# DiltheyLab/MetaMaps

Measured on AMD Instinct MI355X. Metric: Gbp long reads mapped+classified per sec (whole node), miniSeq+H DB, higher is better.
Workload: dtype u32

## Files before the change

metamaps_amd/csrc/mm_env.hpp:

```cpp
#pragma once
#include <unistd.h>
#include <cstdlib>
#include <cstring>
#include <string>

extern "C" char** environ;

namespace mm {

struct EnvSwitch { const char* name; const char* dflt; const char* kind; const char* what; };

inline const EnvSwitch* env_table(size_t* n) {
  static const EnvSwitch T[] = {
    {"MM_STRICT_ENV", "unset", "user", "refuse MM_* variables that are not in this table (mm_ctx_create returns MM_ERR_ARG, the CLI exits 1)"},
    {"MM_CPU_BUDGET", "min(hardware threads, affinity mask, cgroup CPU quota)", "user", "CPUs the process may keep busy: what every thread pool of the library and the CLI is sized from (cpu_budget.hpp)"},
    {"MM_SYNC", "block when the CPU budget is <= 32, else spin", "user", "how a host thread waits for its stream: \"spin\" (hipStreamSynchronize) or \"block\" (sleep on an event created with hipEventBlockingSync)"},
    {"MM_CLI_WORKERS", "4", "user", "worker contexts per GPU that take read batches in turn (= --workers-per-gpu)"},
    {"MM_CLI_BATCH_READS", "100000", "user", "reads per batch handed to a worker"},
    {"MM_CLI_BATCH_MBASES", "256", "user", "... or this many million bases, whichever comes first"},
    {"MM_CLI_MAP_SLOTS", "2", "tuning", "batches per device that may be inside their mapping section at the same time"},
    {"MM_CLI_BLOCK_BYTES", "128 MiB", "tuning", "block size of the block-parallel FASTQ/FASTA parser over an mmap-ed query file"},
    {"MM_CLI_REF_BLOCK_BYTES", "min(group, 256 MiB)", "tuning", "the same for the reference FASTA"},
    {"MM_CLI_REF_GROUP_BASES", "2^30", "test", "bases per upload group of the reference (small groups: the concat path on small inputs)"},
    {"MM_CLI_REF_SEQUENTIAL", "unset", "test", "reference through the sequential kseq-style reader instead of the block parser"},
// ... 13 lines not shown
    {"MM_CLASSIFY_THREADS", "32", "user", "host threads that tokenise the mappings file and format classify's outputs"},
    {"MM_EM_MAX_ITER", "unbounded", "test", "cap on EM iterations in classify (the reference has none)"},
    {"MM_EM_SLICE", "1024", "test", "EM iterations per mm_em_run / mm_em_continue call of classify"},
    {"MM_CLI_TIMING", "unset", "debug", "phase laps of the CLI on stderr (bench.py's e2e legs parse them)"},
    {"MM_CLI_FORMAT_TRACE", "unset", "debug", "per-thread times of the text formatting of a batch on stderr"},
    {"MM_DEVICE_BYTES_CAP", "0 (off)", "test", "the library behaves as if every device had this many bytes: allocations beyond fail, mm_ctx_device_info reports it (placement tests)"},
    {"MM_INDEX_SCALE_MB", "8192", "test", "blocks from this size on are index-scale (pooled per device); a few MB exercise the pool on small inputs"},
    {"MM_NO_SLABS", "unset", "test", "worker buffers are not cut out of pooled index-scale blocks"},
    {"MM_NO_POOL_RESCUE", "unset", "test", "round-3 behaviour: a request the driver refuses hands the whole pool back instead of being served from it"},
    {"MM_ALLOC_TRACE", "unset", "debug", "every block that comes from the driver, with its cost, on stderr"},
    {"MM_CTX_TRACE", "unset", "debug", "phases of mm_ctx_create (HIP initialisation, stream, allocator) on stderr"},
    {"MM_HOST_TIMING", "unset", "debug", "host-side sections of mm_map_batch and of the index build on stderr"},
    {"MM_PACK_SCALAR", "unset", "test", "mm_seqset_upload packs bases with the byte-table loop only (cross-check of the AVX2 path, host_pack.cpp)"},
    {"MM_INDEX_PART_MAX", "2^31 - 2^24 entries", "test", "entries per partition of the hash sort (small values: the partitioned sort + merge on small inputs)"},
    {"MM_DUP_SAT", "65535", "test", "saturation value of the stored same-hash neighbour distances (small values: K5's scan fall-back)"},
    {"MM_EAGER_TIEBREAK", "unset", "test", "resolve every duplicate-hash strand by the reference's std::sort order up front instead of only where a strand vote reads one"},
    {"MM_FORCE_AMB_REDO", "unset", "test", "every read with an unresolved strand goes through the redo path"},
    {"MM_NO_HIT_FILTER", "unset", "test", "K3 without the exact seed-hit pre-filter: every hit of every kept list reaches the sort (parity tests of the raw hit list)"},
    {"MM_NO_FUSED_FILTER", "unset", "test", "K3 as probe_kernel + two-pass hit_filter_kernel for every read (what reads that do not fit the fused kernel take)"},
    {"MM_HF_STAGE_CAP", "auto", "test", "capacity of a read's survivor stage (tiny values: the overflow / re-filter path)"},
    {"MM_HF_WIDE_FROM", "13000", "tuning", "sketch size from which the two-pass filter counts in 32768 position slots instead of 8192"},
    {"MM_SEGSORT_MAX_KEYS", "2^32 - 1", "test", "keys per call of K4's segmented device sort (small values: the split on small inputs)"},
    {"MM_L1_SERIAL", "unset", "test", "K4's L1 merge loop as the literal one-thread-per-read loop (cross-check of the wavefront form)"},
    {"MM_L2_FULL", "unset", "test", "K5 evaluates every window (the literal slide) instead of the exact skip-ahead"},
    {"MM_L2_DENSE_FROM", "13000", "tuning", "sketch size from which K5 runs as l2_codes_kernel + l2_dense_kernel"},
    {"MM_L2_DENSE_NO_STOP", "unset", "test", "dense path without its early stop (every window evaluated)"},
    {"MM_L2_NO_SMALL_GROUPS", "unset", "test", "groups of fewer than three candidates also run as four-wave workgroups (one launch instead of two)"},
    {"MM_L2_HOST_GROUPS", "unset", "test", "candidate groups formed on the host instead of by l2_group_kernel"},
    {"MM_L2_NO_GROUP_SORT", "unset", "test", "K5 workgroups in read order instead of the order of their candidates' positions"},
    {"MM_L2_GROUP_SORT_MIN", "2048", "tuning", "groups from which the launch order is sorted"},
    {"MM_L2_V1", "unset", "test", "K5's 10 kb class through l2_kernel (rank codes per entry) instead of the zone kernel l2z_kernel (mm_l2z.hpp): the cross-check and the A/B"},
    {"MM_L2_V1_LONG", "unset", "test", "the long-read classes (sketches of 3 073 .. 13 000 hashes) through l2_kernel, the 10 kb class through the zone kernel"},
    {"MM_L2_NO_FUSE", "unset", "test", "zone kernel without the band predicted from L1's seed-hit count: its masks always come from a second pass over the stream"},
    {"MM_L2_NO_RANGES", "unset", "test", "the zone kernel's waves search their candidates' index ranges themselves (until round 6) instead of taking them from l2_ranges_kernel (cross-check)"},
    {"MM_L2Z_FORCE_HANDBACK", "unset", "test", "the zone kernel hands every candidate that reaches its band loop to l2_kernel, as its pass-count guard does (the hand-back path against the default)"},
    {"MM_L2Z_WALK_SEARCH", "unset", "test", "the 10 kb zone kernel finds the next block to sweep by the walk one block at a time (the long-read classes' way) instead of by ballots: the same blocks, the cross-check"},
    {"MM_L2Z_DBG", "unset", "debug", "zone kernel writes pivot-minus-estimate and its pass count INSTEAD OF RESULTS (tools/l2z_pivot_hist.py; 2: against the predicted estimate)"},
    {"MM_L2_ONE_STREAM", "unset", "test", "the two launches of K5's 10 kb class one behind the other on the context's stream instead of side by side (auxiliary stream)"},
    {"MM_L2_NO_SLOTS", "unset", "test", "K5 scratch indexed by wave number of the launch instead of per-XCD slots taken and given back"},
    {"MM_L2_SLOTS", "auto (resident waves)", "tuning", "number of K5 scratch slots"},
    {"MM_L2_STOP", "0", "debug", "K5 leaves after phase n WITHOUT RESULTS (tools/l2_stop.py)"},
    {"MM_L2_PHASES", "unset", "debug", "K5 phase clocks into its counters (tools/l2_long_phases.py; the zone kernel has them in a build with -DL2Z_CLOCKS only)"},
    {"MM_MZ_DBG", "0", "debug", "K1 leaves after step n WITHOUT RESULTS (tools/stage_ms.py)"},
    {"MM_HF_DBG", "0", "debug", "two-pass filter leaves after phase n WITHOUT RESULTS"},
    {"MM_SF_PROF", "unset", "debug", "cycle counts per phase of the streaming seed filter on stderr"},
    {"MM_EM_FORCE_COLLECTIVE", "unset", "test", "a one-rank communicator keeps P1-P3' | ncclAllReduce | finalize instead of P1-P3 alone (how one GPU drives the multi-rank path)"},
// ... 40 lines not shown
```

metamaps_amd/csrc/mm_l1.hpp:

```cpp
#pragma once
#include <rocprim/rocprim.hpp>
#include "mm_map.hpp"
#include "mm_l2.hpp"

namespace mm {

template <int IPT>
__global__ void __launch_bounds__(256) sort_hits_radix_kernel(uint64_t* __restrict__ hits, const uint64_t* __restrict__ read_hit_off,
                                                              const int32_t* __restrict__ read_list, int end_bit,
                                                              const uint64_t* __restrict__ stage ,
                                                              const uint64_t* __restrict__ stage_off ) {
  using Sort = rocprim::block_radix_sort<uint64_t, 256, IPT>;
  extern __shared__ __align__(16) unsigned char sort_dyn[];
  typename Sort::storage_type& tmp = *reinterpret_cast<typename Sort::storage_type*>(sort_dyn);
  const int r = read_list[blockIdx.x];
  const uint64_t o = read_hit_off[r];
  const int n = (int)(read_hit_off[r + 1] - o);
  const uint64_t* __restrict__ src = hits + o;
  if (stage) { const uint64_t sb = stage_off[r]; if ((uint64_t)n <= stage_off[r + 1] - sb) src = stage + sb; }
  uint64_t key[IPT];
#pragma unroll
  for (int i = 0; i < IPT; ++i) { const int idx = threadIdx.x * IPT + i; key[i] = idx < n ? src[idx] : ~0ull; }
  Sort().sort(key, tmp, 0, end_bit);
#pragma unroll
  for (int i = 0; i < IPT; ++i) { const int idx = threadIdx.x * IPT + i; if (idx < n) hits[o + idx] = key[i]; }
}

template <bool WRITE>
__global__ void l1_scan_kernel(const uint64_t* __restrict__ hits, const uint64_t* __restrict__ read_hit_off, const int32_t* __restrict__ read_len,
                               const int32_t* __restrict__ min_hits, int64_t n_reads, uint32_t* __restrict__ cand_n,
                               const uint64_t* __restrict__ cand_off, int32_t* __restrict__ cand, int32_t* __restrict__ cand_read) {
  int64_t r = (int64_t)blockIdx.x * blockDim.x + threadIdx.x;
  if (r >= n_reads) return;
  const uint64_t o = read_hit_off[r];
  const int64_t H = (int64_t)(read_hit_off[r + 1] - o);
  const int len = read_len[r];
  int m = min_hits[r]; if (m < 1) m = 1;
  uint32_t nc = 0;
  int lseq = -1, lstart = 0, lend = 0;
  uint64_t wbase = WRITE ? cand_off[r] : 0;
  auto flush = [&]() {
    if (lseq < 0) return;
    if (WRITE) { int32_t* c = cand + 3 * (wbase + nc); c[0] = lseq; c[1] = lstart; c[2] = lend; cand_read[wbase + nc] = (int32_t)r; }
    ++nc;
  };
  for (int64_t i = 0; i + m <= H; ++i) {
    uint64_t a = hits[o + i], b = hits[o + i + m - 1];
    int sa = (int)(a >> 32), sb = (int)(b >> 32);
    int wa = pw_wpos((uint32_t)a), wb = pw_wpos((uint32_t)b);
    if (sa != sb || wb - wa >= len) continue;
    int cs = max(0, wb - len + 1), ce = wa;
    if (lseq == sa && lend >= cs) lend = max(ce, lend);
    else { flush(); lseq = sa; lstart = cs; lend = ce; }
  }
  flush();
  if (!WRITE) cand_n[r] = nc;
}

template <bool WRITE>
__global__ void __launch_bounds__(256) l1_wave_kernel(const uint64_t* __restrict__ hits, const uint64_t* __restrict__ read_hit_off,
                                                      const int32_t* __restrict__ read_len, const int32_t* __restrict__ min_hits, int64_t n_reads,
                                                      uint32_t* __restrict__ cand_n, const uint64_t* __restrict__ cand_off, int32_t* __restrict__ cand,
                                                      int32_t* __restrict__ cand_read, int32_t* __restrict__ cand_hint ) {
  const int64_t r = (int64_t)blockIdx.x * 4 + (threadIdx.x >> 6);
  const int lane = threadIdx.x & 63;
  if (r >= n_reads) return;
  const uint64_t o = read_hit_off[r];
  const int64_t H = (int64_t)(read_hit_off[r + 1] - o);
  const int len = read_len[r];
  int m = min_hits[r]; if (m < 1) m = 1;
  const uint64_t wbase = WRITE ? cand_off[r] : 0;
  int count = 0, prev_seq = -1, prev_wa = 0;
  int64_t open_i = 0;
  for (int64_t base = 0; base + m <= H; base += 64) {
    const int64_t i = base + lane;
    const bool valid = i + m <= H;
    uint64_t a = 0, b = 0;
    if (valid) { a = hits[o + i]; b = hits[o + i + m - 1]; }
    const int sa = (int)(a >> 32), sb = (int)(b >> 32), wa = pw_wpos((uint32_t)a), wb = pw_wpos((uint32_t)b);
    const bool q = valid && sa == sb && wb - wa < len;
    const int cs = max(0, wb - len + 1);
    const uint64_t qm = __ballot(q);
    const uint64_t below = qm & ((1ull << lane) - 1ull);
    const int pl = below ? 63 - __builtin_clzll(below) : 0;
    const int p_seq_l = __shfl(sa, pl, 64), p_wa_l = __shfl(wa, pl, 64);
    const int p_seq = below ? p_seq_l : prev_seq, p_wa = below ? p_wa_l : prev_wa;
    const bool brk = q && !(p_seq == sa && p_wa >= cs);
    const uint64_t bm = __ballot(brk);
    if (WRITE && q) {
      const int k = count + __popcll(bm & ((2ull << lane) - 1ull)) - 1;
      const uint64_t above = lane < 63 ? qm & ~((2ull << lane) - 1ull) : 0ull;
      const bool last = above == 0ull || ((bm >> (__builtin_ctzll(above))) & 1ull);
      int32_t* c = cand + 3 * (wbase + (uint64_t)k);
      if (brk) { c[0] = sa; c[1] = cs; cand_read[wbase + (uint64_t)k] = (int32_t)r; }
      if (last) c[2] = wa;
      if (last && cand_hint) {
        const uint64_t opened = bm & ((2ull << lane) - 1ull);
        const int64_t oi = opened ? base + (63 - __builtin_clzll(opened)) : open_i;
        cand_hint[wbase + (uint64_t)k] = (int32_t)min((int64_t)0x7fffffff, i + m - oi);
      }
    }
    if (bm) open_i = base + (63 - __builtin_clzll(bm));
    count += __popcll(bm);
    if (qm) { const int ll = 63 - __builtin_clzll(qm); prev_seq = __shfl(sa, ll, 64); prev_wa = __shfl(wa, ll, 64); }
  }
  if (!WRITE && lane == 0) cand_n[r] = (uint32_t)count;
}

__global__ void __launch_bounds__(256) l2_group_kernel(const uint64_t* __restrict__ cand_off, const int32_t* __restrict__ sk_n, const int32_t* __restrict__ read_len,
                                                       int64_t n, int min_len_dense, int dense_from, int no_small,
                                                       int32_t* __restrict__ gA0, int32_t* __restrict__ gAn, int32_t* __restrict__ gS0, int32_t* __restrict__ gSn,
                                                       unsigned int* __restrict__ ctr) {
  __shared__ unsigned int bA, bS, bOther, bMax, baseA, baseS;
  if (threadIdx.x == 0) { bA = 0; bS = 0; bOther = 0; bMax = 0; }
  __syncthreads();
  const int64_t r = (int64_t)blockIdx.x * 256 + threadIdx.x;
  uint64_t c_lo = 0, c_hi = 0; int sr = 0; bool mine = false;
  if (r < n) {
    c_lo = cand_off[r]; c_hi = cand_off[r + 1]; sr = sk_n[r];
    const bool dense = sr >= dense_from && sr < L2_SKETCH_LIMIT && read_len[r] >= min_len_dense;
    mine = c_hi > c_lo && sr <= 3072 && !dense;
    if (c_hi > c_lo && !mine) atomicAdd(&bOther, 1u);
  }
  const unsigned ncr = mine ? (unsigned)(c_hi - c_lo) : 0u, nfull = ncr >> 2, rem = ncr & 3u;
  const bool rem_small = rem != 0 && rem <= 2 && !no_small;
  const unsigned a = nfull + ((rem != 0 && !rem_small) ? 1u : 0u), b = rem_small ? 1u : 0u;
  unsigned la = 0, ls = 0;
  if (a) la = atomicAdd(&bA, a);
  if (b) ls = atomicAdd(&bS, b);
// ... 82 lines not shown
```

metamaps_amd/csrc/mm_map.hip:

```cpp
#include "mm_map.hpp"
#include <functional>
#include <memory>
#include "mm_prims.hpp"
#include "mm_l2_core.hpp"
#include "mm_size_classes.hpp"
#include "mm_l2.hpp"
#include "mm_l2z.hpp"
#include "mm_l2_dense.hpp"
#include <cstdlib>
#include <atomic>
#include <thread>
#include "mm_stats.hpp"
#include <algorithm>
#include <numeric>
#include "mm_sketch.hpp"
#include "mm_seed.hpp"
#include "mm_l1.hpp"

namespace mm {

namespace {
struct HostLap {
  const bool on = getenv("MM_HOST_TIMING") != nullptr; std::chrono::steady_clock::time_point t = std::chrono::steady_clock::now();
  void operator()(const char* what) { if (!on) return; const auto n = std::chrono::steady_clock::now(); fprintf(stderr, "host %-28s %8.1f us\n", what, std::chrono::duration<double, std::micro>(n - t).count()); t = n; }
// ... 48 lines not shown
  std::vector<uint8_t> sv; std::vector<int32_t> scnt; std::atomic<int> mismatch{0};
  ~AmbState() { if (bg.joinable()) bg.join(); }
};

namespace {
struct MapSwitches {
  struct OptInt { bool set; int v; };
  static bool on(const char* e) { return e != nullptr; }
  static bool is1(const char* e) { return e && e[0] == '1'; }
  static int num(const char* e, int dflt) { return e ? atoi(e) : dflt; }
  static OptInt opt(const char* e) { return OptInt{e != nullptr, e ? atoi(e) : 0}; }
  const bool eager_tiebreak = on(getenv("MM_EAGER_TIEBREAK"));
  const bool use_filter = !is1(getenv("MM_NO_HIT_FILTER"));
  const bool use_fused = use_filter && !on(getenv("MM_NO_FUSED_FILTER"));
  const int hf_wide_env = num(getenv("MM_HF_WIDE_FROM"), 13000);
  const int hf_wide_from = hf_wide_env > 0 ? hf_wide_env : INT_MAX;
  const OptInt hf_stage_cap = opt(getenv("MM_HF_STAGE_CAP"));
  const int hf_dbg = num(getenv("MM_HF_DBG"), 0);
  const bool sf_prof = on(getenv("MM_SF_PROF"));
  const OptInt sf_grid = opt(getenv("MM_SF_GRID"));
  const OptInt segsort_max_env = opt(getenv("MM_SEGSORT_MAX_KEYS"));
  const uint64_t segsort_max_keys = segsort_max_env.set ? (uint64_t)std::max(segsort_max_env.v, 1) : 0xffffffffull;
  const bool l1_serial = on(getenv("MM_L1_SERIAL"));
  const bool l2_no_fuse = on(getenv("MM_L2_NO_FUSE"));
  const bool l2_no_ranges = on(getenv("MM_L2_NO_RANGES"));
  const bool l2_skip = !is1(getenv("MM_L2_FULL"));
  const int dense_from = num(getenv("MM_L2_DENSE_FROM"), 13000);
  const bool dense_no_stop = on(getenv("MM_L2_DENSE_NO_STOP"));
  const bool no_small_groups = on(getenv("MM_L2_NO_SMALL_GROUPS"));
  const bool dev_groups = l2_skip && !on(getenv("MM_L2_HOST_GROUPS"));
  const bool l2_no_slots = on(getenv("MM_L2_NO_SLOTS"));
  const OptInt l2_slots_env = opt(getenv("MM_L2_SLOTS"));
  const size_t l2_slots = l2_slots_env.set ? ((size_t)std::max(l2_slots_env.v, 1) + 7) / 8 * 8 : 0;
  const bool v2 = !on(getenv("MM_L2_V1"));
  const bool v2_long = v2 && !on(getenv("MM_L2_V1_LONG"));
  const bool sort_groups = !on(getenv("MM_L2_NO_GROUP_SORT"));
  const OptInt group_sort_env = opt(getenv("MM_L2_GROUP_SORT_MIN"));
  const size_t group_sort_from = group_sort_env.set ? (size_t)std::max(group_sort_env.v, 1) : 2048;
  const bool one_stream = on(getenv("MM_L2_ONE_STREAM"));
  const OptInt l2_stop = opt(getenv("MM_L2_STOP"));
  const bool l2_phases = on(getenv("MM_L2_PHASES"));
  const bool force_amb_redo = on(getenv("MM_FORCE_AMB_REDO"));
  const OptInt l2z_dbg = opt(getenv("MM_L2Z_DBG"));
  const bool l2z_force_handback = on(getenv("MM_L2Z_FORCE_HANDBACK"));
  const bool l2z_walk_search = on(getenv("MM_L2Z_WALK_SEARCH"));
  bool has_l2_debug_word() const { return l2_stop.set || l2_phases || force_amb_redo || l2z_dbg.set || l2z_force_handback || l2z_walk_search; }
// ... 22 lines not shown
  const hipStream_t st;
  const MapSwitches sw;
  StageTimer T;
  const int64_t n;
  size_t t_total = 0, t_l1 = 0;
  int64_t total_mz = 0, total_hits = 0, ncand = 0;
  HostLap hl;
  std::vector<uint8_t> h_amb;
  std::function<void()> amb_finish;
  std::vector<int64_t> eager_reads, lazy_reads;
  std::vector<std::unique_ptr<AmbState>> amb_states;
  IndexView IV{};
  DBuf<uint32_t> probe_cnt;
  DBuf<uint64_t> probe_start;
  DBuf<uint64_t> hit_off, scan_tmp;
  DBuf<uint8_t> need_old; DBuf<uint32_t> raw_per_read;
  int64_t n_fused = 0, n_wide = 0;
  uint64_t raw_hits = 0;
  DBuf<unsigned long long> raw_sum;
  DBuf<uint32_t> surv;
  DBuf<uint64_t> stage, stage_off;
  const uint8_t* only = nullptr;
  DBuf<uint32_t> cand_n;
  DBuf<int32_t> cand_hint;
  DBuf<int64_t> cand_rng;
  DBuf<int32_t> d_gA0, d_gAn, d_gS0, d_gSn;
  DBuf<unsigned int> grp_ctr;
  std::vector<int32_t> listG; int smG = 0;
  DBuf<unsigned long long> counters;
  DBuf<int32_t> ovf;
  DBuf<unsigned int> ovf_n;
  DBuf<uint8_t> amb_used;
  uint8_t* amb_used_p = nullptr;
  struct SkipClasses {
    DBuf<unsigned int> slot_flags;
    DBuf<int32_t> big;
    DBuf<unsigned int> big_n;
    std::vector<int32_t> gA0, gAn, gB0, gBn, gD0, gDn, listC, gS0, gSn;
    int smA = 0, smB = 0, smC = 0, smD = 0;
    std::vector<int32_t> listL; int smL = 0;
    std::vector<unsigned int> gctr = std::vector<unsigned int>(4, 0);
    size_t nA = 0, nS = 0;
    DBuf<int32_t> d_gB0, d_gBn, d_listC, d_gD0, d_gDn;
    int64_t n_fallback = 0, n_big = 0, n_redo = 0;
  };
  std::unique_ptr<SkipClasses> sk;
// ... 48 lines not shown
  void sketch() {
    if (M->sketch_donor) return;
    size_t t_sk = T.begin(&M->stats.ms_sketch);
    static_assert(ipt_list_is<4, 6, 8, 10, 12, 16, 20, 24, 32, 40, 48, 64>(SKETCH_IPTS), "the dispatch below lists the classes of mm_size_classes.hpp");
    uint64_t big_seen = 0;
    HostLap hl;
    const ReadBins RB = bin_reads(n, N_SKETCH_CLASSES, [&](int64_t r) -> int {
      const uint64_t c = hoff()[(size_t)r + 1] - hoff()[(size_t)r];
      big_seen |= (uint64_t)(c > SKETCH_LDS_MAX);
      return sketch_class_index(c);
    });
    const bool any_big = big_seen != 0;
    {
      hl("K2 bin");
      DBuf<int32_t> list(std::max<size_t>(RB.order.size(), 1));
      list.upload(RB.order.data(), RB.order.size(), st);
      hl("K2 list upload");
      size_t at = 0;
      for (auto& run : RB.runs) {
        const unsigned nb = (unsigned)run.second;
        const int32_t* lp = list.p + at;
        dispatch<4, 6, 8, 10, 12, 16, 20, 24, 32, 40, 48, 64>(SKETCH_IPTS[run.first], [&](auto ipt_tag) {
          constexpr int IPT = decltype(ipt_tag)::value;
          using SortT = rocprim::block_radix_sort<uint32_t, 256, IPT, uint16_t>;
          using ScanT = rocprim::block_scan<int, 256>;
          const size_t lds = std::max(sizeof(typename SortT::storage_type), sizeof(typename ScanT::storage_type)) + 16;
          if (lds > 48 * 1024) MM_HIP(hipFuncSetAttribute((const void*)sketch_radix_kernel<IPT>, hipFuncAttributeMaxDynamicSharedMemorySize, (int)lds));
          sketch_radix_kernel<IPT><<<dim3(nb), dim3(256), lds, st>>>(M->mz.rec.p, M->mz.off.p, lp, M->sk_hash.p, M->sk_strand.p, M->sk_n.p, M->amb.p);
        });
        MM_KERNEL_CHECK();
        at += run.second;
      }
      hl("K2 launches");
      MM_HIP(mm::stream_sync(st));
      hl("K2 sync (kernels)");
    }
    if (any_big) sketch_big_segmented();
    T.end(t_sk);
  }

  void sketch_big_segmented() {
    std::vector<int32_t> big; std::vector<uint64_t> koff{0};
    for (int64_t r = 0; r < n; ++r) { const uint64_t c = hoff()[(size_t)r + 1] - hoff()[(size_t)r]; if (c > SKETCH_LDS_MAX) { big.push_back((int32_t)r); koff.push_back(koff.back() + c); } }
    const size_t nb = big.size(); const uint64_t nk = koff.back();
    MM_REQUIRE(nk < ((uint64_t)1 << 32), MM_ERR_LIMIT, "more than 2^32 minimizers of reads beyond 16384 minimizers in one batch");
    DBuf<int32_t> d_big(nb); d_big.upload(big.data(), nb, st);
    DBuf<uint64_t> d_koff(nb + 1); d_koff.upload(koff.data(), nb + 1, st);
    DBuf<uint64_t> keys((size_t)nk), sorted((size_t)nk);
    sketch_keys_kernel<<<dim3((unsigned)nb), dim3(256), 0, st>>>(M->mz.rec.p, M->mz.off.p, d_big.p, d_koff.p, keys.p);
// ... 216 lines not shown
    const size_t t_sf = T.begin(&M->stats.ms_hit_filter);
    if (sf_prof.p)
      seed_filter_stream_kernel<true><<<dim3((unsigned)sf_grid), dim3(SF_THREADS), lds, st>>>(IV, M->sk_hash.p, M->mz.off.p, M->sk_n.p, M->d_read_len.p, M->min_hits.p, surv.p, stage.p, stage_off.p,
                                                                         need_old.p, reinterpret_cast<const uint32_t*>(need_old.p), raw_per_read.p, (int)n, sf_ticket.p, sf_prof.p);
    else
      seed_filter_stream_kernel<false><<<dim3((unsigned)sf_grid), dim3(SF_THREADS), lds, st>>>(IV, M->sk_hash.p, M->mz.off.p, M->sk_n.p, M->d_read_len.p, M->min_hits.p, surv.p, stage.p, stage_off.p,
                                                                         need_old.p, reinterpret_cast<const uint32_t*>(need_old.p), raw_per_read.p, (int)n, sf_ticket.p, nullptr);
    MM_KERNEL_CHECK();
    T.end(t_sf);
    if (sf_prof.p) {
      auto h = sf_prof.to_host(st);
      const double tot = (double)std::accumulate(h.begin(), h.end(), 0ull);
      fprintf(stderr, "MM_SF_PROF share of cycles: zero+top %.3f | next head + resolve %.3f | scan %.3f | lists+count %.3f | window sums+alive+issue %.3f | phase 2 %.3f | survivors+end %.3f | total %.3g cycles over %d workgroups\n",
              h[0] / tot, (h[1] + h[7]) / tot, h[2] / tot, (h[3] + h[8]) / tot, (h[4] + h[9] + h[10] + h[11]) / tot, (h[5] + h[12]) / tot, h[6] / tot, tot, sf_grid);
      fprintf(stderr, "MM_SF_PROF in detail: top %.3f | first answers + second probes issued %.3f, their answers %.3f | scan %.3f | pieces loaded, counted, parked %.3f, next hashes asked for + barrier %.3f | "
                      "window sums %.3f, alive %.3f, barrier %.3f, hashes there + look-ups issued %.3f | bit tests + slots %.3f, barrier %.3f | survivors+end %.3f\n",
              h[0] / tot, h[7] / tot, h[1] / tot, h[2] / tot, h[8] / tot, h[3] / tot, h[9] / tot, h[10] / tot, h[4] / tot, h[11] / tot, h[12] / tot, h[5] / tot, h[6] / tot);
    }
  }

  int64_t hits_of(int64_t r) const { return (int64_t)(M->h_read_hit_off[(size_t)r + 1] - M->h_read_hit_off[(size_t)r]); }

  void sort_hits() {
    if (total_hits > 0) {
      const size_t t_sh = T.begin(&M->stats.ms_sort_hits);
      hl("K4 hits alloc + emit launch");
      int key_bits = 32; while (key_bits < 64 && ((int64_t)1 << (key_bits - 32)) < I->n_contigs) ++key_bits;
      if (sort_hits_radix(key_bits)) sort_hits_segmented(key_bits);
      T.end(t_sh);
    }
    hl("K4 launches + sync");
  }

  bool sort_hits_radix(int key_bits) {
    static_assert(ipt_list_is<1, 2, 3, 4, 6, 8, 12, 16>(HIT_SORT_IPTS), "the dispatch below lists the classes of mm_size_classes.hpp");
    uint64_t left_seen = 0;
    const ReadBins RB = bin_reads(n, N_HIT_SORT_CLASSES, [&](int64_t r) -> int {
      const uint64_t c = (uint64_t)hits_of(r);
      left_seen |= (uint64_t)(c > HIT_SORT_LDS_MAX);
      return hit_sort_class_index(c);
    });
    hl("K4 bin");
    DBuf<int32_t> list(std::max<size_t>(RB.order.size(), 1));
    list.upload(RB.order.data(), RB.order.size(), st);
    hl("K4 list upload");
    size_t at = 0;
    for (auto& run : RB.runs) {
      const int32_t* lp = list.p + at;
      dispatch<1, 2, 3, 4, 6, 8, 12, 16>(HIT_SORT_IPTS[run.first], [&](auto tag) {
        constexpr int IPT = decltype(tag)::value;
        using SortT = rocprim::block_radix_sort<uint64_t, 256, IPT>;
        const size_t lds = sizeof(typename SortT::storage_type) + 16;
        if (lds > 48 * 1024) MM_HIP(hipFuncSetAttribute((const void*)sort_hits_radix_kernel<IPT>, hipFuncAttributeMaxDynamicSharedMemorySize, (int)lds));
        sort_hits_radix_kernel<IPT><<<dim3((unsigned)run.second), dim3(256), lds, st>>>(M->hits.p, M->read_hit_off.p, lp, key_bits, sw.use_filter ? stage.p : nullptr, sw.use_filter ? stage_off.p : nullptr);
      });
      MM_KERNEL_CHECK();
      at += run.second;
    }
    MM_HIP(mm::stream_sync(st));
    return left_seen != 0;
  }

  void sort_hits_segmented(int key_bits) {
    const uint64_t max_keys = sw.segsort_max_keys;
    std::vector<int32_t> seg_reads;
    std::vector<uint64_t> hb, he, cb, ce;
    std::vector<size_t> run_at{0};
    uint64_t in_run = 0, longest_run = 0;
    for (int64_t r = 0; r < n; ++r) {
      const uint64_t c = (uint64_t)hits_of(r);
      if (c <= HIT_SORT_LDS_MAX) continue;
      MM_REQUIRE(c < max_keys, MM_ERR_LIMIT, "one read has more seed hits than a segmented sort takes (2^32 - 1, or MM_SEGSORT_MAX_KEYS)");
      if (in_run + c >= max_keys) { run_at.push_back(seg_reads.size()); in_run = 0; }
      seg_reads.push_back((int32_t)r);
      hb.push_back(M->h_read_hit_off[(size_t)r]); he.push_back(M->h_read_hit_off[(size_t)r + 1]);
      cb.push_back(in_run); in_run += c; ce.push_back(in_run);
      longest_run = std::max(longest_run, in_run);
    }
    const size_t ns = seg_reads.size();
    run_at.push_back(ns);
    const bool compact = run_at.size() > 2 || 2 * longest_run <= (uint64_t)total_hits || (uint64_t)total_hits >= max_keys;
    DBuf<uint64_t> d_hb(ns), d_he(ns), d_cb(ns), d_ce(ns);
    d_hb.upload(hb.data(), ns, st); d_he.upload(he.data(), ns, st);
    auto seg_sort = [&](uint64_t* in, uint64_t* out, uint64_t count, size_t nseg, uint64_t* begins, uint64_t* ends) {
      with_scratch([&](void* t, size_t& b) { return rocprim::segmented_radix_sort_keys(t, b, in, out, (unsigned int)count, (unsigned int)nseg, begins, ends, 0, key_bits, st); });
    };
    if (compact) {
      d_cb.upload(cb.data(), ns, st); d_ce.upload(ce.data(), ns, st);
      DBuf<uint64_t> packed((size_t)longest_run), sorted((size_t)longest_run);
      for (size_t k = 0; k + 1 < run_at.size(); ++k) {
        const size_t i0 = run_at[k], nr = run_at[k + 1] - i0;
        move_ranges_kernel<<<dim3((unsigned)nr), dim3(256), 0, st>>>(M->hits.p, d_hb.p + i0, d_he.p + i0, packed.p, d_cb.p + i0);
        MM_KERNEL_CHECK();
        seg_sort(packed.p, sorted.p, ce[i0 + nr - 1], nr, d_cb.p + i0, d_ce.p + i0);
        move_ranges_kernel<<<dim3((unsigned)nr), dim3(256), 0, st>>>(sorted.p, d_cb.p + i0, d_ce.p + i0, M->hits.p, d_hb.p + i0);
        MM_KERNEL_CHECK();
      }
      MM_HIP(mm::stream_sync(st));
    } else {
      DBuf<uint64_t> sorted((size_t)total_hits);
      seg_sort(M->hits.p, sorted.p, (uint64_t)total_hits, ns, d_hb.p, d_he.p);
      move_ranges_kernel<<<dim3((unsigned)ns), dim3(256), 0, st>>>(sorted.p, d_hb.p, d_he.p, M->hits.p, d_hb.p);
      MM_KERNEL_CHECK();
      MM_HIP(mm::stream_sync(st));
    }
  }

  void l1_candidates() {
    t_l1 = T.begin(&M->stats.ms_l1_scan);
    cand_n.alloc((size_t)n + 1); cand_n.zero(st);
    M->cand_off.alloc((size_t)n + 2);
    const unsigned rblk = (unsigned)ceil_div(std::max<int64_t>(n, 1), 128);
    if (n > 0) {
      if (sw.l1_serial) l1_scan_kernel<false><<<dim3(rblk), dim3(128), 0, st>>>(M->hits.p, M->read_hit_off.p, M->d_read_len.p, M->min_hits.p, n, cand_n.p, nullptr, nullptr, nullptr);
      else l1_wave_kernel<false><<<dim3((unsigned)ceil_div(n, 4)), dim3(256), 0, st>>>(M->hits.p, M->read_hit_off.p, M->d_read_len.p, M->min_hits.p, n, cand_n.p, nullptr, nullptr, nullptr, nullptr);
      MM_KERNEL_CHECK();
    }
    exclusive_scan_u32_u64(cand_n.p, n, M->cand_off.p, scan_tmp, st);
    M->h_cand_off = M->cand_off.to_host(st, (size_t)n + 1);
    hl("L1 count + cand_off download");
    ncand = (int64_t)M->h_cand_off[(size_t)n];
    M->n_cand = ncand;
    M->stats.n_candidates = ncand;
    MM_REQUIRE(ncand < (1LL << 31), MM_ERR_LIMIT, "more than 2^31 L1 candidates in one batch");
    M->cand.alloc((size_t)std::max<int64_t>(3 * ncand, 1));
    M->cand_read.alloc((size_t)std::max<int64_t>(ncand, 1));
    M->l2.alloc((size_t)std::max<int64_t>(ncand, 1));
    cand_hint.alloc((size_t)std::max<int64_t>(ncand, 1));
    const bool no_hint = sw.l1_serial || sw.l2_no_fuse;
    if (no_hint) cand_hint.zero(st);
    M->rec_off.alloc((size_t)n + 1);
    if (ncand == 0) return;
    if (sw.l1_serial) l1_scan_kernel<true><<<dim3(rblk), dim3(128), 0, st>>>(M->hits.p, M->read_hit_off.p, M->d_read_len.p, M->min_hits.p, n, nullptr, M->cand_off.p, M->cand.p, M->cand_read.p);
    else l1_wave_kernel<true><<<dim3((unsigned)ceil_div(n, 4)), dim3(256), 0, st>>>(M->hits.p, M->read_hit_off.p, M->d_read_len.p, M->min_hits.p, n, nullptr, M->cand_off.p, M->cand.p, M->cand_read.p, no_hint ? nullptr : cand_hint.p);
    MM_KERNEL_CHECK();
    T.end(t_l1);
  }

  template <bool SKIP, typename CNT, int NW, int NWQ>
  void launch_l2(size_t grid, hipStream_t s, int sm, const int32_t* g0, const int32_t* gn, const int32_t* list, uint8_t* amb_ptr, void* codes, uint8_t* masks, int n_slots) {
    const size_t lds = l2_lds_bytes<CNT>(sm, SKIP, NW, NWQ);
    set_lds((const void*)l2_kernel<SKIP, CNT, NW, NWQ>, lds);
    l2_kernel<SKIP, CNT, NW, NWQ><<<dim3((unsigned)grid), dim3(64 * NW), lds, s>>>(IV, M->cand.p, M->cand_read.p, M->sk_hash.p, M->sk_strand.p,
        M->mz.off.p, M->sk_n.p, M->d_read_len.p, M->accept_min.p, P.k, P.w, sm, M->l2.p, counters.p, g0, gn, list, SKIP ? ovf.p : nullptr, SKIP ? ovf_n.p : nullptr, amb_ptr,
        codes, masks, SKIP ? slot_flags_p() : nullptr, n_slots);
    MM_KERNEL_CHECK();
  }
  template <int NW, int NWQ, bool QLDS>
  void launch_l2z(size_t grid, hipStream_t s, int sm, const int32_t* g0, const int32_t* gn, void* lists, uint8_t* masks, int n_slots) {
    const int bbl = l2z_bloom_log2(sm);
    const size_t lds = l2z_lds_bytes(sm, NWQ, QLDS, bbl, NW);
    set_lds((const void*)l2z_kernel<NW, NWQ, QLDS>, lds);
    l2z_kernel<NW, NWQ, QLDS><<<dim3((unsigned)grid), dim3(64 * NW), lds, s>>>(IV, M->cand.p, M->cand_read.p, M->sk_hash.p, M->sk_strand.p, M->mz.off.p, M->sk_n.p, M->d_read_len.p,
        M->accept_min.p, P.k, P.w, sm, bbl, M->l2.p, counters.p, g0, gn, ovf.p, ovf_n.p, sk->big.p, sk->big_n.p, amb_used_p, (uint32_t*)lists, masks, slot_flags_p(), n_slots, cand_hint.p, cand_rng.p);
    MM_KERNEL_CHECK();
  }
  void launch_l2_wide(const int32_t* list, size_t nl, int sm, uint8_t* amb_ptr) {
// ... 346 lines not shown
```

metamaps_amd/csrc/mm_sketch.hpp:

```cpp
#pragma once
#include <rocprim/rocprim.hpp>
#include "mm_map.hpp"

namespace mm {

template <int IPT>
__global__ void __launch_bounds__(256) sketch_radix_kernel(const Rec* __restrict__ rec, const uint64_t* __restrict__ off,
                                                           const int32_t* __restrict__ read_list, uint32_t* __restrict__ sk_hash,
                                                           uint8_t* __restrict__ sk_strand, int32_t* __restrict__ sk_n, uint8_t* __restrict__ amb) {
  using Sort = rocprim::block_radix_sort<uint32_t, 256, IPT, uint16_t>;
  using Scan = rocprim::block_scan<int, 256>;
  union Tmp { typename Sort::storage_type sort; typename Scan::storage_type scan; };
  extern __shared__ __align__(16) unsigned char sketch_dyn[];
  Tmp& tmp = *reinterpret_cast<Tmp*>(sketch_dyn);
  __shared__ uint32_t last_key[256];
  __shared__ uint8_t last_st[256];
  __shared__ int s_amb;
  const int r = read_list[blockIdx.x];
  const uint64_t o = off[r];
  const int n = (int)(off[r + 1] - o);
  const int t = threadIdx.x;
  uint32_t key[IPT]; uint16_t val[IPT];
#pragma unroll
  for (int i = 0; i < IPT; ++i) { const int idx = t * IPT + i; key[i] = idx < n ? rec[o + idx].hash : 0xffffffffu; val[i] = (uint16_t)idx; }
  if (t == 0) s_amb = 0;
  Sort().sort(key, val, tmp.sort);
  uint8_t stv[IPT];
#pragma unroll
  for (int i = 0; i < IPT; ++i) stv[i] = (t * IPT + i < n) ? (uint8_t)(rec[o + val[i]].pw & PW_STRAND) : 0;
  last_key[t] = key[IPT - 1]; last_st[t] = stv[IPT - 1];
  __syncthreads();
  int nfirst = 0; bool first[IPT]; bool ambig = false;
#pragma unroll
  for (int i = 0; i < IPT; ++i) {
// ... 94 lines not shown
```

Baseline: 25.83.

## Fuse L1 candidate scan into per-read hit sort kernel via LDS slots

```diff
diff --git a/metamaps_amd/csrc/mm_env.hpp b/metamaps_amd/csrc/mm_env.hpp
--- a/metamaps_amd/csrc/mm_env.hpp
+++ b/metamaps_amd/csrc/mm_env.hpp
@@ -59,6 +59,7 @@
     {"MM_HF_WIDE_FROM", "13000", "tuning", "sketch size from which the two-pass filter counts in 32768 position slots instead of 8192"},
     {"MM_SEGSORT_MAX_KEYS", "2^32 - 1", "test", "keys per call of K4's segmented device sort (small values: the split on small inputs)"},
     {"MM_L1_SERIAL", "unset", "test", "K4's L1 merge loop as the literal one-thread-per-read loop (cross-check of the wavefront form)"},
+    {"MM_L1_TWO_LAUNCH", "unset", "test", "K4's L1 as its two wavefront kernels (count, then write) over every read instead of inside the hit sort's kernels: the cross-check and the A/B"},
     {"MM_L2_FULL", "unset", "test", "K5 evaluates every window (the literal slide) instead of the exact skip-ahead"},
     {"MM_L2_DENSE_FROM", "13000", "tuning", "sketch size from which K5 runs as l2_codes_kernel + l2_dense_kernel"},
     {"MM_L2_DENSE_NO_STOP", "unset", "test", "dense path without its early stop (every window evaluated)"},
diff --git a/metamaps_amd/csrc/mm_l1.hpp b/metamaps_amd/csrc/mm_l1.hpp
--- a/metamaps_amd/csrc/mm_l1.hpp
+++ b/metamaps_amd/csrc/mm_l1.hpp
@@ -4,27 +4,6 @@
 #include "mm_l2.hpp"
 
 namespace mm {
-
-template <int IPT>
-__global__ void __launch_bounds__(256) sort_hits_radix_kernel(uint64_t* __restrict__ hits, const uint64_t* __restrict__ read_hit_off,
-                                                              const int32_t* __restrict__ read_list, int end_bit,
-                                                              const uint64_t* __restrict__ stage ,
-                                                              const uint64_t* __restrict__ stage_off ) {
-  using Sort = rocprim::block_radix_sort<uint64_t, 256, IPT>;
-  extern __shared__ __align__(16) unsigned char sort_dyn[];
-  typename Sort::storage_type& tmp = *reinterpret_cast<typename Sort::storage_type*>(sort_dyn);
-  const int r = read_list[blockIdx.x];
-  const uint64_t o = read_hit_off[r];
-  const int n = (int)(read_hit_off[r + 1] - o);
-  const uint64_t* __restrict__ src = hits + o;
-  if (stage) { const uint64_t sb = stage_off[r]; if ((uint64_t)n <= stage_off[r + 1] - sb) src = stage + sb; }
-  uint64_t key[IPT];
-#pragma unroll
-  for (int i = 0; i < IPT; ++i) { const int idx = threadIdx.x * IPT + i; key[i] = idx < n ? src[idx] : ~0ull; }
-  Sort().sort(key, tmp, 0, end_bit);
-#pragma unroll
-  for (int i = 0; i < IPT; ++i) { const int idx = threadIdx.x * IPT + i; if (idx < n) hits[o + idx] = key[i]; }
-}
 
 template <bool WRITE>
 __global__ void l1_scan_kernel(const uint64_t* __restrict__ hits, const uint64_t* __restrict__ read_hit_off, const int32_t* __restrict__ read_len,
@@ -57,26 +36,15 @@
   if (!WRITE) cand_n[r] = nc;
 }
 
-template <bool WRITE>
-__global__ void __launch_bounds__(256) l1_wave_kernel(const uint64_t* __restrict__ hits, const uint64_t* __restrict__ read_hit_off,
-                                                      const int32_t* __restrict__ read_len, const int32_t* __restrict__ min_hits, int64_t n_reads,
-                                                      uint32_t* __restrict__ cand_n, const uint64_t* __restrict__ cand_off, int32_t* __restrict__ cand,
-                                                      int32_t* __restrict__ cand_read, int32_t* __restrict__ cand_hint ) {
-  const int64_t r = (int64_t)blockIdx.x * 4 + (threadIdx.x >> 6);
-  const int lane = threadIdx.x & 63;
-  if (r >= n_reads) return;
-  const uint64_t o = read_hit_off[r];
-  const int64_t H = (int64_t)(read_hit_off[r + 1] - o);
-  const int len = read_len[r];
-  int m = min_hits[r]; if (m < 1) m = 1;
-  const uint64_t wbase = WRITE ? cand_off[r] : 0;
+template <bool WRITE, typename Sink>
+__device__ __forceinline__ int l1_wave_loop(const uint64_t* __restrict__ hits, int64_t H, int len, int m, int lane, Sink&& sink) {
   int count = 0, prev_seq = -1, prev_wa = 0;
   int64_t open_i = 0;
   for (int64_t base = 0; base + m <= H; base += 64) {
     const int64_t i = base + lane;
     const bool valid = i + m <= H;
     uint64_t a = 0, b = 0;
-    if (valid) { a = hits[o + i]; b = hits[o + i + m - 1]; }
+    if (valid) { a = hits[i]; b = hits[i + m - 1]; }
     const int sa = (int)(a >> 32), sb = (int)(b >> 32), wa = pw_wpos((uint32_t)a), wb = pw_wpos((uint32_t)b);
     const bool q = valid && sa == sb && wb - wa < len;
     const int cs = max(0, wb - len + 1);
@@ -91,20 +59,116 @@
       const int k = count + __popcll(bm & ((2ull << lane) - 1ull)) - 1;
       const uint64_t above = lane < 63 ? qm & ~((2ull << lane) - 1ull) : 0ull;
       const bool last = above == 0ull || ((bm >> (__builtin_ctzll(above))) & 1ull);
-      int32_t* c = cand + 3 * (wbase + (uint64_t)k);
-      if (brk) { c[0] = sa; c[1] = cs; cand_read[wbase + (uint64_t)k] = (int32_t)r; }
-      if (last) c[2] = wa;
-      if (last && cand_hint) {
+      if (brk) sink.open(k, sa, cs);
+      if (last) {
+        sink.close(k, wa);
         const uint64_t opened = bm & ((2ull << lane) - 1ull);
         const int64_t oi = opened ? base + (63 - __builtin_clzll(opened)) : open_i;
-        cand_hint[wbase + (uint64_t)k] = (int32_t)min((int64_t)0x7fffffff, i + m - oi);
+        sink.hint(k, (int32_t)min((int64_t)0x7fffffff, i + m - oi));
       }
     }
     if (bm) open_i = base + (63 - __builtin_clzll(bm));
     count += __popcll(bm);
     if (qm) { const int ll = 63 - __builtin_clzll(qm); prev_seq = __shfl(sa, ll, 64); prev_wa = __shfl(wa, ll, 64); }
   }
-  if (!WRITE && lane == 0) cand_n[r] = (uint32_t)count;
+  return count;
+}
+struct L1NoSink {
+  __device__ void open(int, int, int) const {}
+  __device__ void close(int, int) const {}
+  __device__ void hint(int, int32_t) const {}
+};
+struct L1CandSink {
+  int32_t* cand; int32_t* cand_read; int32_t* cand_hint ; uint64_t wbase; int32_t r;
+  __device__ void open(int k, int seq, int cs) const { int32_t* c = cand + 3 * (wbase + (uint64_t)k); c[0] = seq; c[1] = cs; cand_read[wbase + (uint64_t)k] = r; }
+  __device__ void close(int k, int wa) const { cand[3 * (wbase + (uint64_t)k) + 2] = wa; }
+  __device__ void hint(int k, int32_t v) const { if (cand_hint) cand_hint[wbase + (uint64_t)k] = v; }
+};
+struct L1SlotSink {
+  int32_t* slot;
+  __device__ void open(int k, int seq, int cs) const { slot[4 * k] = seq; slot[4 * k + 1] = cs; }
+  __device__ void close(int k, int wa) const { slot[4 * k + 2] = wa; }
+  __device__ void hint(int k, int32_t v) const { slot[4 * k + 3] = v; }
+};
+
+#ifndef HIT_SORT_RADIX_BITS
+#define HIT_SORT_RADIX_BITS 0
+#endif
+template <int IPT> using HitSort = rocprim::block_radix_sort<uint64_t, 256, IPT, rocprim::empty_type, 1, 1, HIT_SORT_RADIX_BITS>;
+template <int IPT> constexpr size_t hit_sort_lds_bytes() {
+  return (sizeof(typename HitSort<IPT>::storage_type) > 256 * IPT * sizeof(uint64_t) ? sizeof(typename HitSort<IPT>::storage_type) : 256 * IPT * sizeof(uint64_t)) + 16;
+}
+
+template <int IPT>
+__global__ void __launch_bounds__(256) sort_hits_radix_kernel(uint64_t* __restrict__ hits, const uint64_t* __restrict__ read_hit_off,
+                                                              const int32_t* __restrict__ read_list, int end_bit,
+                                                              const uint64_t* __restrict__ stage ,
+                                                              const uint64_t* __restrict__ stage_off ,
+                                                              const int32_t* __restrict__ read_len, const int32_t* __restrict__ min_hits,
+                                                              uint32_t* __restrict__ cand_n, int32_t* __restrict__ l1_slots ) {
+  using Sort = HitSort<IPT>;
+  extern __shared__ __align__(16) unsigned char sort_dyn[];
+  typename Sort::storage_type& tmp = *reinterpret_cast<typename Sort::storage_type*>(sort_dyn);
+  const int r = read_list[blockIdx.x];
+  const uint64_t o = read_hit_off[r];
+  const int n = (int)(read_hit_off[r + 1] - o);
+  const uint64_t* __restrict__ src = hits + o;
+  if (stage) { const uint64_t sb = stage_off[r]; if ((uint64_t)n <= stage_off[r + 1] - sb) src = stage + sb; }
+  int len = 0, m = 1;
+  if (l1_slots) { len = read_len[r]; m = max(min_hits[r], 1); }
+  uint64_t key[IPT];
+#pragma unroll
+  for (int i = 0; i < IPT; ++i) { const int idx = threadIdx.x * IPT + i; key[i] = idx < n ? src[idx] : ~0ull; }
+  Sort().sort(key, tmp, PW_SHIFT, end_bit);
+#pragma unroll
+  for (int i = 0; i < IPT; ++i) { const int idx = threadIdx.x * IPT + i; if (idx < n) hits[o + idx] = key[i]; }
+  if (!l1_slots) return;
+  uint64_t* const sorted = reinterpret_cast<uint64_t*>(sort_dyn);
+  __syncthreads();
+#pragma unroll
+  for (int i = 0; i < IPT; ++i) { const int idx = threadIdx.x * IPT + i; if (idx < n) sorted[idx] = key[i]; }
+  __syncthreads();
+  if (threadIdx.x >= 64) return;
+  const int count = l1_wave_loop<true>(sorted, n, len, m, (int)threadIdx.x, L1SlotSink{l1_slots + 4 * o});
+  if (threadIdx.x == 0) cand_n[r] = (uint32_t)count;
+}
+
+__global__ void __launch_bounds__(256) l1_place_kernel(const int32_t* __restrict__ l1_slots, const uint64_t* __restrict__ read_hit_off, const uint64_t* __restrict__ cand_off,
+                                                       int64_t n_reads, uint64_t max_hits, int32_t* __restrict__ cand, int32_t* __restrict__ cand_read,
+                                                       int32_t* __restrict__ cand_hint ) {
+  const int64_t r = (int64_t)blockIdx.x * 256 + threadIdx.x;
+  if (r >= n_reads) return;
+  const uint64_t o = read_hit_off[r], H = read_hit_off[r + 1] - o;
+  if (H < 2 || H > max_hits) return;
+  const uint64_t c0 = cand_off[r], nc = cand_off[r + 1] - c0;
+  const int4* __restrict__ s = reinterpret_cast<const int4*>(l1_slots) + o;
+  for (uint64_t k = 0; k < nc; ++k) {
+    const int4 v = s[k];
+    int32_t* c = cand + 3 * (c0 + k);
+    c[0] = v.x; c[1] = v.y; c[2] = v.z; cand_read[c0 + k] = (int32_t)r;
+    if (cand_hint) cand_hint[c0 + k] = v.w;
+  }
+}
+
+template <bool WRITE>
+__global__ void __launch_bounds__(256) l1_wave_kernel(const uint64_t* __restrict__ hits, const uint64_t* __restrict__ read_hit_off,
+                                                      const int32_t* __restrict__ read_len, const int32_t* __restrict__ min_hits,
+                                                      const int32_t* __restrict__ read_list, int64_t n_reads,
+                                                      uint32_t* __restrict__ cand_n, const uint64_t* __restrict__ cand_off, int32_t* __restrict__ cand,
+                                                      int32_t* __restrict__ cand_read, int32_t* __restrict__ cand_hint ) {
+  const int64_t at = (int64_t)blockIdx.x * 4 + (threadIdx.x >> 6);
+  const int lane = threadIdx.x & 63;
+  if (at >= n_reads) return;
+  const int64_t r = read_list ? (int64_t)read_list[at] : at;
+  const uint64_t o = read_hit_off[r];
+  const int64_t H = (int64_t)(read_hit_off[r + 1] - o);
+  const int len = read_len[r];
+  int m = min_hits[r]; if (m < 1) m = 1;
+  if (WRITE) l1_wave_loop<true>(hits + o, H, len, m, lane, L1CandSink{cand, cand_read, cand_hint, cand_off[r], (int32_t)r});
+  else {
+    const int count = l1_wave_loop<false>(hits + o, H, len, m, lane, L1NoSink{});
+    if (lane == 0) cand_n[r] = (uint32_t)count;
+  }
 }
 
 __global__ void __launch_bounds__(256) l2_group_kernel(const uint64_t* __restrict__ cand_off, const int32_t* __restrict__ sk_n, const int32_t* __restrict__ read_len,
diff --git a/metamaps_amd/csrc/mm_map.hip b/metamaps_amd/csrc/mm_map.hip
--- a/metamaps_amd/csrc/mm_map.hip
+++ b/metamaps_amd/csrc/mm_map.hip
@@ -94,6 +94,7 @@
   const OptInt segsort_max_env = opt(getenv("MM_SEGSORT_MAX_KEYS"));
   const uint64_t segsort_max_keys = segsort_max_env.set ? (uint64_t)std::max(segsort_max_env.v, 1) : 0xffffffffull;
   const bool l1_serial = on(getenv("MM_L1_SERIAL"));
+  const bool l1_fused = !l1_serial && !on(getenv("MM_L1_TWO_LAUNCH"));
   const bool l2_no_fuse = on(getenv("MM_L2_NO_FUSE"));
   const bool l2_no_ranges = on(getenv("MM_L2_NO_RANGES"));
   const bool l2_skip = !is1(getenv("MM_L2_FULL"));
@@ -162,6 +163,8 @@
   DBuf<uint64_t> stage, stage_off;
   const uint8_t* only = nullptr;
   DBuf<uint32_t> cand_n;
+  DBuf<int32_t> l1_slots;
+  DBuf<int32_t> l1_rest; size_t n_l1_rest = 0;
   DBuf<int32_t> cand_hint;
   DBuf<int64_t> cand_rng;
   DBuf<int32_t> d_gA0, d_gAn, d_gS0, d_gSn;
@@ -256,9 +259,7 @@
         const int32_t* lp = list.p + at;
         dispatch<4, 6, 8, 10, 12, 16, 20, 24, 32, 40, 48, 64>(SKETCH_IPTS[run.first], [&](auto ipt_tag) {
           constexpr int IPT = decltype(ipt_tag)::value;
-          using SortT = rocprim::block_radix_sort<uint32_t, 256, IPT, uint16_t>;
-          using ScanT = rocprim::block_scan<int, 256>;
-          const size_t lds = std::max(sizeof(typename SortT::storage_type), sizeof(typename ScanT::storage_type)) + 16;
+          const size_t lds = sketch_lds_bytes<IPT>();
           if (lds > 48 * 1024) MM_HIP(hipFuncSetAttribute((const void*)sketch_radix_kernel<IPT>, hipFuncAttributeMaxDynamicSharedMemorySize, (int)lds));
           sketch_radix_kernel<IPT><<<dim3(nb), dim3(256), lds, st>>>(M->mz.rec.p, M->mz.off.p, lp, M->sk_hash.p, M->sk_strand.p, M->sk_n.p, M->amb.p);
         });
@@ -521,7 +522,9 @@
   int64_t hits_of(int64_t r) const { return (int64_t)(M->h_read_hit_off[(size_t)r + 1] - M->h_read_hit_off[(size_t)r]); }
 
   void sort_hits() {
+    cand_n.alloc((size_t)n + 1); cand_n.zero(st);
     if (total_hits > 0) {
+      if (sw.l1_fused) l1_slots.alloc(4 * (size_t)total_hits);
       const size_t t_sh = T.begin(&M->stats.ms_sort_hits);
       hl("K4 hits alloc + emit launch");
       int key_bits = 32; while (key_bits < 64 && ((int64_t)1 << (key_bits - 32)) < I->n_contigs) ++key_bits;
@@ -534,11 +537,16 @@
   bool sort_hits_radix(int key_bits) {
     static_assert(ipt_list_is<1, 2, 3, 4, 6, 8, 12, 16>(HIT_SORT_IPTS), "the dispatch below lists the classes of mm_size_classes.hpp");
     uint64_t left_seen = 0;
+    std::vector<int32_t> rest;
     const ReadBins RB = bin_reads(n, N_HIT_SORT_CLASSES, [&](int64_t r) -> int {
       const uint64_t c = (uint64_t)hits_of(r);
       left_seen |= (uint64_t)(c > HIT_SORT_LDS_MAX);
-      return hit_sort_class_index(c);
+      const int cls = hit_sort_class_index(c);
+      if (cls == N_HIT_SORT_CLASSES && c > 0 && sw.l1_fused) rest.push_back((int32_t)r);
+      return cls;
     });
+    n_l1_rest = rest.size();
+    if (n_l1_rest) { l1_rest.alloc(n_l1_rest); l1_rest.upload(rest.data(), n_l1_rest, st); }
     hl("K4 bin");
     DBuf<int32_t> list(std::max<size_t>(RB.order.size(), 1));
     list.upload(RB.order.data(), RB.order.size(), st);
@@ -548,10 +556,10 @@
       const int32_t* lp = list.p + at;
       dispatch<1, 2, 3, 4, 6, 8, 12, 16>(HIT_SORT_IPTS[run.first], [&](auto tag) {
         constexpr int IPT = decltype(tag)::value;
-        using SortT = rocprim::block_radix_sort<uint64_t, 256, IPT>;
-        const size_t lds = sizeof(typename SortT::storage_type) + 16;
+        const size_t lds = hit_sort_lds_bytes<IPT>();
         if (lds > 48 * 1024) MM_HIP(hipFuncSetAttribute((const void*)sort_hits_radix_kernel<IPT>, hipFuncAttributeMaxDynamicSharedMemorySize, (int)lds));
-        sort_hits_radix_kernel<IPT><<<dim3((unsigned)run.second), dim3(256), lds, st>>>(M->hits.p, M->read_hit_off.p, lp, key_bits, sw.use_filter ? stage.p : nullptr, sw.use_filter ? stage_off.p : nullptr);
+        sort_hits_radix_kernel<IPT><<<dim3((unsigned)run.second), dim3(256), lds, st>>>(M->hits.p, M->read_hit_off.p, lp, key_bits, sw.use_filter ? stage.p : nullptr, sw.use_filter ? stage_off.p : nullptr,
+                                                                                     M->d_read_len.p, M->min_hits.p, cand_n.p, l1_slots.p);
       });
       MM_KERNEL_CHECK();
       at += run.second;
@@ -582,7 +590,7 @@
     DBuf<uint64_t> d_hb(ns), d_he(ns), d_cb(ns), d_ce(ns);
     d_hb.upload(hb.data(), ns, st); d_he.upload(he.data(), ns, st);
     auto seg_sort = [&](uint64_t* in, uint64_t* out, uint64_t count, size_t nseg, uint64_t* begins, uint64_t* ends) {
-      with_scratch([&](void* t, size_t& b) { return rocprim::segmented_radix_sort_keys(t, b, in, out, (unsigned int)count, (unsigned int)nseg, begins, ends, 0, key_bits, st); });
+      with_scratch([&](void* t, size_t& b) { return rocprim::segmented_radix_sort_keys(t, b, in, out, (unsigned int)count, (unsigned int)nseg, begins, ends, PW_SHIFT, key_bits, st); });
     };
     if (compact) {
       d_cb.upload(cb.data(), ns, st); d_ce.upload(ce.data(), ns, st);
@@ -607,12 +615,13 @@
 
   void l1_candidates() {
     t_l1 = T.begin(&M->stats.ms_l1_scan);
-    cand_n.alloc((size_t)n + 1); cand_n.zero(st);
     M->cand_off.alloc((size_t)n + 2);
     const unsigned rblk = (unsigned)ceil_div(std::max<int64_t>(n, 1), 128);
+    const int32_t* const wave_list = sw.l1_fused ? l1_rest.p : nullptr;
+    const int64_t n_wave = sw.l1_fused ? (int64_t)n_l1_rest : n;
     if (n > 0) {
       if (sw.l1_serial) l1_scan_kernel<false><<<dim3(rblk), dim3(128), 0, st>>>(M->hits.p, M->read_hit_off.p, M->d_read_len.p, M->min_hits.p, n, cand_n.p, nullptr, nullptr, nullptr);
-      else l1_wave_kernel<false><<<dim3((unsigned)ceil_div(n, 4)), dim3(256), 0, st>>>(M->hits.p, M->read_hit_off.p, M->d_read_len.p, M->min_hits.p, n, cand_n.p, nullptr, nullptr, nullptr, nullptr);
+      else if (n_wave > 0) l1_wave_kernel<false><<<dim3((unsigned)ceil_div(n_wave, 4)), dim3(256), 0, st>>>(M->hits.p, M->read_hit_off.p, M->d_read_len.p, M->min_hits.p, wave_list, n_wave, cand_n.p, nullptr, nullptr, nullptr, nullptr);
       MM_KERNEL_CHECK();
     }
     exclusive_scan_u32_u64(cand_n.p, n, M->cand_off.p, scan_tmp, st);
@@ -631,7 +640,12 @@
     M->rec_off.alloc((size_t)n + 1);
     if (ncand == 0) return;
     if (sw.l1_serial) l1_scan_kernel<true><<<dim3(rblk), dim3(128), 0, st>>>(M->hits.p, M->read_hit_off.p, M->d_read_len.p, M->min_hits.p, n, nullptr, M->cand_off.p, M->cand.p, M->cand_read.p);
-    else l1_wave_kernel<true><<<dim3((unsigned)ceil_div(n, 4)), dim3(256), 0, st>>>(M->hits.p, M->read_hit_off.p, M->d_read_len.p, M->min_hits.p, n, nullptr, M->cand_off.p, M->cand.p, M->cand_read.p, no_hint ? nullptr : cand_hint.p);
+    else {
+      if (sw.l1_fused && l1_slots.p)
+        l1_place_kernel<<<dim3((unsigned)ceil_div(n, 256)), dim3(256), 0, st>>>(l1_slots.p, M->read_hit_off.p, M->cand_off.p, n, (uint64_t)HIT_SORT_LDS_MAX, M->cand.p, M->cand_read.p, no_hint ? nullptr : cand_hint.p);
+      if (n_wave > 0)
+        l1_wave_kernel<true><<<dim3((unsigned)ceil_div(n_wave, 4)), dim3(256), 0, st>>>(M->hits.p, M->read_hit_off.p, M->d_read_len.p, M->min_hits.p, wave_list, n_wave, nullptr, M->cand_off.p, M->cand.p, M->cand_read.p, no_hint ? nullptr : cand_hint.p);
+    }
     MM_KERNEL_CHECK();
     T.end(t_l1);
   }
diff --git a/metamaps_amd/csrc/mm_sketch.hpp b/metamaps_amd/csrc/mm_sketch.hpp
--- a/metamaps_amd/csrc/mm_sketch.hpp
+++ b/metamaps_amd/csrc/mm_sketch.hpp
@@ -4,12 +4,20 @@
 
 namespace mm {
 
+#ifndef SKETCH_RADIX_BITS
+#define SKETCH_RADIX_BITS 0
+#endif
+template <int IPT> using SketchSort = rocprim::block_radix_sort<uint32_t, 256, IPT, uint16_t, 1, 1, SKETCH_RADIX_BITS>;
+using SketchScan = rocprim::block_scan<int, 256>;
+template <int IPT> constexpr size_t sketch_lds_bytes() {
+  return (sizeof(typename SketchSort<IPT>::storage_type) > sizeof(typename SketchScan::storage_type) ? sizeof(typename SketchSort<IPT>::storage_type) : sizeof(typename SketchScan::storage_type)) + 16;
+}
 template <int IPT>
 __global__ void __launch_bounds__(256) sketch_radix_kernel(const Rec* __restrict__ rec, const uint64_t* __restrict__ off,
                                                            const int32_t* __restrict__ read_list, uint32_t* __restrict__ sk_hash,
                                                            uint8_t* __restrict__ sk_strand, int32_t* __restrict__ sk_n, uint8_t* __restrict__ amb) {
-  using Sort = rocprim::block_radix_sort<uint32_t, 256, IPT, uint16_t>;
-  using Scan = rocprim::block_scan<int, 256>;
+  using Sort = SketchSort<IPT>;
+  using Scan = SketchScan;
   union Tmp { typename Sort::storage_type sort; typename Scan::storage_type scan; };
   extern __shared__ __align__(16) unsigned char sketch_dyn[];
   Tmp& tmp = *reinterpret_cast<Tmp*>(sketch_dyn);
```

New measurement: 25.99, median of 6. No clear change (+0.6%).
